# askerlee/segtran

Measured on NVIDIA H100. Metric: voxels/sec fwd+bwd Segtran3d BraTS 112^3 bs=4 hot path, higher is better.
Workload: dtype tf32

## Files before the change

### include/segtran_b200.h

```cpp
#ifndef SEGTRAN_B200_H_
#define SEGTRAN_B200_H_

#include <stddef.h>
#include <stdint.h>

#ifdef __cplusplus
extern "C" {
#endif

#define SX_VERSION 1

enum { SX_F32 = 0, SX_BF16 = 1 };
enum { SX_OP_TF32 = 0, SX_OP_BF16 = 1 };
enum { SX_MAJOR_K = 0, SX_MAJOR_MN = 1 };
enum { SX_BIAS_NONE = 0, SX_BIAS_N = 1, SX_BIAS_M = 2 };
enum { SX_ACT_NONE = 0, SX_ACT_GELU = 1,
       SX_ACT_GELU_BWD = 2  };

int sx_version(void);
const char* sx_last_error(void);
int sx_device_info(int* sm_count, int* cc_major, int* cc_minor);

typedef struct {
  const void* ptr;
// ... 12 lines not shown
  int32_t c_dtype;
  int32_t round_tf32;
  int64_t ldc, c_stride_z0, c_stride_z1;
  float alpha;
  int32_t bias_mode;
  const float* bias;
  int64_t bias_stride_z0, bias_stride_z1;
  int32_t act;
  int32_t accumulate;
  void* preact;
  int32_t split_k;
  int32_t _pad2;
  float* amax;
  float drop_p;
  uint32_t _pad3;
  uint64_t drop_seed;
  const uint64_t* drop_seed_dev;
  const float* addend;
  float* part;
  int64_t part_floats;
} sx_gemm_args;

int sx_gemm(const sx_gemm_args* args, void* stream);

typedef struct {
  const float* table;
  int32_t pd, R;
  int32_t grid[3];
  float w;
} sx_posbias;

typedef struct {
  int32_t B, M, U1, U2, d;
  int32_t round_tf32;
  const float* Q;
  int64_t q_ld, q_bstride;
  const float* K;
  int64_t k_ld, k_bstride;
  float alpha, clip;
  float* P;
  float* S;
  int64_t ldp;
  float* lse;
  float* rowmax;
  float* stat;
  float* diag;
// ... 203 lines not shown
```

### segtran_b200/_lib.py

```python
from __future__ import annotations

import ctypes as C
import os

_HERE = os.path.dirname(os.path.abspath(__file__))
LIB_PATH = os.path.join(_HERE, "libsegtran_b200.so")

SX_F32, SX_BF16 = 0, 1
SX_OP_TF32, SX_OP_BF16 = 0, 1
SX_MAJOR_K, SX_MAJOR_MN = 0, 1
SX_BIAS_NONE, SX_BIAS_N, SX_BIAS_M = 0, 1, 2
SX_ACT_NONE, SX_ACT_GELU, SX_ACT_GELU_BWD = 0, 1, 2
SX_SCHED_WARMUP_LINEAR, SX_SCHED_WARMUP_CONSTANT = 0, 1
SX_CONSIST_BCE, SX_CONSIST_MARGIN = 0, 1
SX_HEAD_DMAP_NONE, SX_HEAD_DMAP_INTERP, SX_HEAD_DMAP_UNFOLD = 0, 1, 2


class SxError(RuntimeError):
    pass


class sx_operand(C.Structure):
    _fields_ = [("ptr", C.c_void_p), ("major", C.c_int32), ("_pad", C.c_int32), ("ld", C.c_int64),
                ("stride_z0", C.c_int64), ("stride_z1", C.c_int64)]


class sx_gemm_args(C.Structure):
    _fields_ = [("op_dtype", C.c_int32), ("M", C.c_int32), ("N", C.c_int32), ("K", C.c_int32), ("Z0", C.c_int32),
                ("Z1", C.c_int32), ("A", sx_operand), ("B", sx_operand), ("C", C.c_void_p), ("c_dtype", C.c_int32),
                ("round_tf32", C.c_int32), ("ldc", C.c_int64), ("c_stride_z0", C.c_int64), ("c_stride_z1", C.c_int64),
                ("alpha", C.c_float), ("bias_mode", C.c_int32), ("bias", C.c_void_p), ("bias_stride_z0", C.c_int64),
                ("bias_stride_z1", C.c_int64), ("act", C.c_int32), ("accumulate", C.c_int32), ("preact", C.c_void_p),
                ("split_k", C.c_int32), ("_pad2", C.c_int32), ("amax", C.c_void_p), ("drop_p", C.c_float),
                ("_pad3", C.c_uint32), ("drop_seed", C.c_uint64), ("drop_seed_dev", C.c_void_p), ("addend", C.c_void_p),
                ("part", C.c_void_p), ("part_floats", C.c_int64)]


class sx_posbias(C.Structure):
    _fields_ = [("table", C.c_void_p), ("pd", C.c_int32), ("R", C.c_int32), ("grid", C.c_int32 * 3), ("w", C.c_float)]


class sx_attn_probs_args(C.Structure):
    _fields_ = [("B", C.c_int32), ("M", C.c_int32), ("U1", C.c_int32), ("U2", C.c_int32), ("d", C.c_int32),
                ("round_tf32", C.c_int32), ("Q", C.c_void_p), ("q_ld", C.c_int64), ("q_bstride", C.c_int64),
                ("K", C.c_void_p), ("k_ld", C.c_int64), ("k_bstride", C.c_int64), ("alpha", C.c_float),
                ("clip", C.c_float), ("P", C.c_void_p), ("S", C.c_void_p), ("ldp", C.c_int64), ("lse", C.c_void_p),
                ("rowmax", C.c_void_p), ("stat", C.c_void_p), ("diag", C.c_void_p), ("drop_p", C.c_float),
                ("_pad", C.c_uint32), ("drop_seed", C.c_uint64), ("drop_seed_dev", C.c_void_p), ("posbias", sx_posbias)]


class sx_consist_args(C.Structure):
    _fields_ = [("B", C.c_int32), ("N", C.c_int32), ("A", C.c_int32), ("K", C.c_int32), ("variant", C.c_int32),
                ("round_r", C.c_int32), ("Xo", C.c_void_p), ("xo_ld", C.c_int64), ("xo_bstride", C.c_int64),
                ("Xt", C.c_void_p), ("xt_ld", C.c_int64), ("xt_bstride", C.c_int64), ("X", C.c_void_p),
                ("x_ld", C.c_int64), ("x_bstride", C.c_int64), ("F", C.c_void_p), ("mu", C.c_void_p), ("R", C.c_void_p),
                ("ldr", C.c_int64), ("out", C.c_void_p), ("cap", C.c_void_p), ("cap_scale", C.c_float),
                ("_pad", C.c_int32), ("part", C.c_void_p), ("part_floats", C.c_int64)]


class sx_head_dropout_args(C.Structure):
    _fields_ = [("src", C.c_void_p), ("B", C.c_int32), ("Fs", C.c_int32), ("Ds", C.c_int32), ("Fo", C.c_int32),
                ("HW", C.c_int64), ("Dk", C.c_int32), ("dmap", C.c_int32), ("K", C.c_int32), ("_pad", C.c_int32),
                ("Wc", C.c_void_p), ("bc", C.c_void_p), ("p", C.c_float), ("_pad2", C.c_uint32), ("seed", C.c_uint64),
                ("seed_dev", C.c_void_p), ("part", C.c_void_p), ("part_floats", C.c_int64)]


class sx_resample_grid(C.Structure):
    _fields_ = [("lin", C.c_int32 * 3), ("lout", C.c_int32 * 3), ("ratio", C.c_float * 3)]


_P, _I, _L, _F, _U64, _D = C.c_void_p, C.c_int32, C.c_int64, C.c_float, C.c_uint64, C.c_double

_PROTOS = {
    "sx_gemm": [C.POINTER(sx_gemm_args), _P],
    "sx_gemm_debug_set": [C.c_char_p, _L],
    "sx_attn_probs_fwd": [C.POINTER(sx_attn_probs_args), _P],
    "sx_attn_consist_fwd": [C.POINTER(sx_consist_args), _P],
    "sx_attn_consist_bwd": [C.POINTER(sx_consist_args), _P, _P, _I, _I, _L, _L, _P, _P, _P, _L, _L, _P],
    "sx_clamp_if": [_P, _L, _I, _L, _P, _F, _P, _L, _P, _L, _P],
    "sx_reduce_max": [_P, _L, _P, _P],
    "sx_pos_lsinu_fwd": [_P, _P, _L, _I, _P, _P, _I, _P, _P],
    "sx_pos_lsinu_bwd": [_P, _P, _L, _I, _P, _P, _I, _P, _P, _P, _P, _P, _L, _P],
    "sx_prologue_fwd": [_P, _L, _I, _I, _P, _P, _P, _I, _L, _F, _P, _F, _U64, _P, _P, _I, _P, _P],
    "sx_prologue_bwd": [_P, _P, _L, _I, _I, _P, _P, _P, _I, _L, _F, _P, _F, _U64, _P, _P, _P, _P, _P, _P, _P, _P, _L, _P],
    "sx_softmax_fwd": [_P, _L, _I, _L, _P, _F, _F, _U64, _P, _P, _L, _I, _P, _P, _P],
    "sx_softmax_bwd": [_P, _L, _P, _L, _P, _L, _I, _P, _F, _F, _U64, _P, _L, _P, _L, _I, _P],
    "sx_softmax_posbias_fwd": [_P, _L, _I, _L, _P, _F, _F, _U64, _P, _P, _L, _I, _P, _P, C.POINTER(sx_posbias), _P],
    "sx_softmax_posbias_bwd": [_P, _L, _P, _L, _P, _L, _I, _P, _F, _F, _U64, _P, _L, _P, _L, _I, C.POINTER(sx_posbias),
                               _P, _P, _L, _P],
    "sx_layernorm_fwd": [_P, _L, _I, _P, _P, _P, _I, _P, _P],
    "sx_layernorm_bwd": [_P, _P, _L, _I, _P, _P, _P, _I, _P, _P, _P, _L, _P],
    "sx_ln_softaggr_fwd": [_P, _I, _I, _I, _I, _P, _P, _P, _P, _F, _U64, _P, _P, _P, _P, _P],
    "sx_ln_softaggr_bwd": [_P, _P, _I, _I, _I, _I, _P, _P, _P, _F, _U64, _P, _P, _P, _P, _I, _P, _P, _P, _P, _P, _L, _P],
    "sx_softaggr_fwd": [_P, _I, _I, _I, _I, _P, _P, _P, _P, _P],
    "sx_softaggr_bwd": [_P, _P, _I, _I, _I, _I, _P, _P, _P, _P, _P],
    "sx_gelu_bwd": [_P, _P, _L, _F, _U64, _P, _P, _I, _P],
    "sx_seed_derive": [_P, _U64, _P, _P],
# ... 48 lines not shown
    global _lib
    if _lib is None:
        if not os.path.isfile(LIB_PATH):
            raise SxError("segtran_b200: %s is missing - run `python -c 'import __graft_entry__ as g; g.build()'` "
                          "or `make` at the repo root (there is no CPU / PyTorch fallback)" % LIB_PATH)
        l = C.CDLL(LIB_PATH)
        l.sx_version.restype = C.c_int
        l.sx_last_error.restype = C.c_char_p
        l.sx_device_info.argtypes = [C.POINTER(C.c_int)] * 3
        l.sx_device_info.restype = C.c_int
        for name, at in _PROTOS.items():
            f = getattr(l, name)
            f.argtypes = at
            f.restype = C.c_int
        _lib = l
    return _lib


def check(rc, what):
    if rc != 0:
        raise SxError("%s failed (rc=%d): %s" % (what, rc, lib().sx_last_error().decode("utf-8", "replace")))


_LAUNCHES = {"sx_pos_lsinu_bwd": 3, "sx_ln_softaggr_bwd": 2, "sx_prologue_bwd": 3, "sx_layernorm_bwd": 3, "sx_gemm_debug_set": 0,
             "sx_attn_probs_fwd": 2, "sx_colsum_batched": 2, "sx_dot": 2, "sx_head_contract_bwd_weight": 2,
             "sx_softmax_posbias_bwd": 2, "sx_attn_consist_fwd": 2, "sx_head_dropout_bwd": 2, "sx_edt_sq": 3}
launch_count = 0
_hook = None


def set_hook(h):
    global _hook
    _hook = h


def call(name, *args):
    global launch_count
    launch_count += _LAUNCHES.get(name, 1)
    if _hook is None:
        check(getattr(lib(), name)(*args), name)
    else:
        with _hook(name, args):
            check(getattr(lib(), name)(*args), name)
```

### segtran_b200/csrc/sx_gemm.cu

```cuda
#include <algorithm>
#include <string>

#include "sx_common.cuh"
#include "sx_tc.cuh"

namespace {
using namespace sxtc;

constexpr int NUM_THREADS = 384;
constexpr int STAGES = 4;
constexpr int XPOSE_WARPS = 3;
constexpr int BN_WIDE = 256;

template <int ES, bool A_MN, bool B_MN, int BN_T>
struct Plan {
  static_assert(BN_T == BN || (BN_T == BN_WIDE && ES == 4 && !A_MN && !B_MN),
                "sx_gemm: the 256-column tile is instantiated for K-major tf32 operands only");
  static constexpr int B_BYTES = BN_T * BKB;
  static constexpr int STAGE_BYTES = A_STAGE_BYTES + B_BYTES;
  static constexpr bool XA = ES == 4 && A_MN, XB = ES == 4 && B_MN;
  static constexpr bool XPOSE = XA || XB;
  static constexpr int RAW_BYTES = (XA ? A_STAGE_BYTES : 0) + (XB ? B_STAGE_BYTES : 0);
  static constexpr int RAW_SLOTS = !XPOSE ? 0 : (XA && XB ? 3 : 4);
  static constexpr int DIRECT_BYTES = STAGE_BYTES - RAW_BYTES;
  static constexpr int SMEM = STAGES * STAGE_BYTES + RAW_SLOTS * RAW_BYTES + 1024  + 256 ;
  static_assert(SMEM <= 227 * 1024, "sx_gemm: shared memory plan exceeds 227 KB");
  static_assert(!XPOSE || (A_STAGE_BYTES == 16384 && B_STAGE_BYTES == 16384 && BM == 128 && BN == 128),
                "sx_gemm: the transposer assumes 128-row, 16 KB tf32 operand tiles");
};

struct GemmParams {
  int M, N, K, Z0, Z1;
  int tiles_m, tiles_n, split_k, kb_per_split, num_kb, total_tiles;
  int z1_loop;
  float* part;
  int a_uses_z0, a_uses_z1, b_uses_z0, b_uses_z1;
  void* C;
  int c_bf16;
  int round_tf32;
  int c_vec_ok;
  long long ldc, c_sz0, c_sz1;
  float alpha;
  int bias_mode;
  const float* bias;
  long long bias_sz0, bias_sz1;
  int act;
  int accumulate;
  void* preact;
  float* amax;
  float drop_p;
  unsigned long long drop_seed;
  const unsigned long long* drop_seed_dev;
  const float* addend;
  int stream_out;
};

__device__ __forceinline__ void xpose_load(uint32_t src, int b, float4 (&v)[4]) {
  const int c = b & 7, kc = c ^ ((b >> 3) & 7);
  const uint32_t s = src + (b >> 6) * 4096;
#pragma unroll
  for (int e = 0; e < 4; ++e) {
    const int k = 4 * kc + e;
    asm volatile("ld.shared.v4.f32 {%0, %1, %2, %3}, [%4];"
                 : "=f"(v[e].x), "=f"(v[e].y), "=f"(v[e].z), "=f"(v[e].w)
                 : "r"(s + k * 128 + ((c ^ (k & 7)) << 4)) : "memory");
  }
}
__device__ __forceinline__ void xpose_store(uint32_t dst, int b, const float4 (&v)[4]) {
  const int c = b & 7, kc = c ^ ((b >> 3) & 7);
  const int r0 = (b >> 6) * 32 + 4 * c;
  auto st = [&](int i, float x, float y, float z, float w) {
    asm volatile("st.shared.v4.f32 [%0], {%1, %2, %3, %4};"
                 ::"r"(dst + (r0 + i) * 128 + ((kc ^ ((r0 + i) & 7)) << 4)), "f"(x), "f"(y), "f"(z), "f"(w) : "memory");
  };
  st(0, v[0].x, v[1].x, v[2].x, v[3].x);
  st(1, v[0].y, v[1].y, v[2].y, v[3].y);
  st(2, v[0].z, v[1].z, v[2].z, v[3].z);
  st(3, v[0].w, v[1].w, v[2].w, v[3].w);
}

template <int ES, bool A_MN, bool B_MN, int BN_T>
__global__ void __launch_bounds__(NUM_THREADS, 1)
sx_gemm_kernel(const __grid_constant__ CUtensorMap tmA, const __grid_constant__ CUtensorMap tmB, const GemmParams p) {
  using PL = Plan<ES, A_MN, B_MN, BN_T>;
  constexpr bool kTF32 = (ES == 4);
  constexpr bool WIDE = BN_T == BN_WIDE;
  constexpr int STAGE_BYTES = PL::STAGE_BYTES;
  constexpr bool XA = PL::XA, XB = PL::XB;
  constexpr int BK = BKB / ES;
  constexpr int MN_BOX = BKB / ES;
  constexpr int MN_BOX_BYTES = BK * BKB;
  constexpr int KSTEPS = 4;

  extern __shared__ uint8_t smem_raw[];
  uint8_t* smem = reinterpret_cast<uint8_t*>((reinterpret_cast<uintptr_t>(smem_raw) + 1023) & ~uintptr_t(1023));
  uint8_t* raw = smem + STAGES * STAGE_BYTES;
  uint64_t* bars = reinterpret_cast<uint64_t*>(raw + PL::RAW_SLOTS * PL::RAW_BYTES);
  uint64_t* full_bar = bars;
  uint64_t* empty_bar = bars + STAGES;
  uint64_t* raw_full = bars + 2 * STAGES;
  uint64_t* raw_empty = raw_full + PL::RAW_SLOTS;

  const int warp = threadIdx.x >> 5;
  const int lane = threadIdx.x & 31;
  const int wg = threadIdx.x >> 7;

  if (threadIdx.x == 0) {
    sx::tma_prefetch_desc(&tmA);
    sx::tma_prefetch_desc(&tmB);
    for (int s = 0; s < STAGES; ++s) {
      sx::mbar_init(&full_bar[s], (PL::DIRECT_BYTES ? 1 : 0) + (PL::XPOSE ? XPOSE_WARPS : 0));
      sx::mbar_init(&empty_bar[s], 2);
    }
    for (int s = 0; s < PL::RAW_SLOTS; ++s) {
      sx::mbar_init(&raw_full[s], 1);
      sx::mbar_init(&raw_empty[s], XPOSE_WARPS);
    }
    sx::fence_barrier_init();
  }
  __syncthreads();

  auto decode = [&](int t, int& z0, int& z1, int& mb, int& nb, int& ks) {
    nb = t % p.tiles_n; t /= p.tiles_n;
    mb = t % p.tiles_m; t /= p.tiles_m;
// ... 302 lines not shown
      if (p.amax) {
#pragma unroll
        for (int h = 0; h < 2; ++h)
          if (row0 + 8 * h + tr < p.M) {
#pragma unroll
            for (int j = 0; j < 4; ++j)
#pragma unroll
              for (int e = 0; e < 2; ++e)
                if (col0 + 8 * j + tc + e < p.N) tmax = fmaxf(tmax, f[4 * j + 2 * h + e]);
          }
      }
      if (!WIDE && p.split_k > 1) {
        float* pt = p.part + ((((long long)z1 * p.Z0 + z0) * p.tiles_m + mb) * p.tiles_n + nb) * p.split_k * (BM * BN) +
                    (long long)ks * (BM * BN);
#pragma unroll
        for (int h = 0; h < 2; ++h)
#pragma unroll
          for (int j = 0; j < 4; ++j)
            *reinterpret_cast<float2*>(pt + (row0 - mb * BM + 8 * h + tr) * BN + (col0 - nb * BN) + 8 * j + tc) =
                make_float2(f[4 * j + 2 * h], f[4 * j + 2 * h + 1]);
      } else {
        store_frag(p.C, f, zoff, row0, col0, p.accumulate != 0);
      }
      if constexpr (WIDE) {
#pragma unroll
        for (int i = 0; i < BN_T / 2 - 16; ++i) acc[i] = acc[i + 16];
      }
    }
    if (p.amax) {
      tmax = sx::warp_max(tmax);
      if (lane == 0 && tmax > -3.0e38f) sx::atomic_max_float(p.amax, tmax);
    }
  }
}

__global__ void split_reduce_kernel(const GemmParams p) {
  const long long total = (long long)p.total_tiles / p.split_k * (BM * BN);
  for (long long i = (long long)blockIdx.x * blockDim.x + threadIdx.x; i < total; i += (long long)gridDim.x * blockDim.x) {
    const int e = (int)(i % (BM * BN));
    long long t = i / (BM * BN);
    const int nb = (int)(t % p.tiles_n); t /= p.tiles_n;
    const int mb = (int)(t % p.tiles_m); t /= p.tiles_m;
    const int z0 = (int)(t % p.Z0), z1 = (int)(t / p.Z0);
    const int row = mb * BM + e / BN, col = nb * BN + e % BN;
    if (row >= p.M || col >= p.N) continue;
    const float* pt = p.part + (i / (BM * BN)) * p.split_k * (BM * BN) + e;
// ... 14 lines not shown
  kern<<<grid, NUM_THREADS, bytes, st>>>(ta, tb, p);
  SX_CHECK_CUDA(cudaGetLastError());
  if (p.split_k > 1) {
    const long long n = (long long)p.total_tiles / p.split_k * (BM * BN);
    split_reduce_kernel<<<(int)std::min<long long>(sx_ceil_div(n, 256), 65535), 256, 0, st>>>(p);
    SX_CHECK_CUDA(cudaGetLastError());
  }
  return 0;
}

}

extern "C" int sx_gemm_debug_set(const char* key, int64_t value) {
  std::string k(key);
  if (k == "max_ctas") g_max_ctas = value;
  else if (k == "wide_tiles") g_wide_tiles = value < 0 ? -1 : (value ? 1 : 0);
  else {
    sx_set_error("sx_gemm_debug_set: unknown key %s", key);
    return -1;
  }
  return 0;
}

extern "C" int sx_gemm(const sx_gemm_args* a, void* stream) {
  SX_REQUIRE(a != nullptr, "sx_gemm: null args");
  SX_REQUIRE(a->M > 0 && a->N > 0 && a->K > 0 && a->Z0 > 0 && a->Z1 > 0, "sx_gemm: bad shape M=%d N=%d K=%d Z=%dx%d",
             a->M, a->N, a->K, a->Z0, a->Z1);
  SX_REQUIRE(a->op_dtype == SX_OP_TF32 || a->op_dtype == SX_OP_BF16, "sx_gemm: bad op_dtype %d", a->op_dtype);
  SX_REQUIRE(a->C != nullptr && a->A.ptr != nullptr && a->B.ptr != nullptr, "sx_gemm: null pointer");
  const int es = a->op_dtype == SX_OP_TF32 ? 4 : 2;
  const int bk = BKB / es;
  const int sms = sm_count_cached();
  SX_REQUIRE(sms > 0, "sx_gemm: no CUDA device (this library has no CPU fallback)");

  GemmParams p{};
  p.M = a->M; p.N = a->N; p.K = a->K; p.Z0 = a->Z0; p.Z1 = a->Z1;
  p.tiles_m = sx_ceil_div(a->M, BM);
  p.tiles_n = sx_ceil_div(a->N, BN);
  p.num_kb = sx_ceil_div(a->K, bk);
  const bool fold_z1 = a->Z1 > 1 && a->c_stride_z1 == 0;
  SX_REQUIRE(!fold_z1 || (a->accumulate && !a->bias && !a->addend && a->act == SX_ACT_NONE && !a->preact && a->drop_p == 0.f),
             "sx_gemm: a z1-reduced output needs accumulate=1 and a linear epilogue without bias");
  p.z1_loop = fold_z1 ? a->Z1 : 1;
  p.Z1 = fold_z1 ? 1 : a->Z1;
  int split = a->split_k < 1 ? 1 : a->split_k;
  if (split > p.num_kb) split = p.num_kb;
  {
// ... 14 lines not shown
  const bool wide_legal = es == 4 && !amn && !bmn && p.split_k == 1;
  const long long wide_tt = (long long)p.tiles_m * sx_ceil_div(a->N, BN_WIDE) * a->Z0 * p.Z1;
  const bool wide = wide_legal && (g_wide_tiles == 1 || (g_wide_tiles < 0 && a->N > BN && 2 * wide_tt > sms));
  if (wide) p.tiles_n = sx_ceil_div(a->N, BN_WIDE);
  const long long tt = (long long)p.tiles_m * p.tiles_n * p.split_k * a->Z0 * p.Z1;
  SX_REQUIRE(tt < (1ll << 30), "sx_gemm: too many tiles");
  p.total_tiles = (int)tt;
  p.a_uses_z0 = a->A.stride_z0 != 0; p.a_uses_z1 = a->A.stride_z1 != 0;
  p.b_uses_z0 = a->B.stride_z0 != 0; p.b_uses_z1 = a->B.stride_z1 != 0;
  p.C = a->C; p.c_bf16 = a->c_dtype == SX_BF16; p.round_tf32 = a->round_tf32;
  p.ldc = a->ldc; p.c_sz0 = a->c_stride_z0; p.c_sz1 = a->c_stride_z1;
  p.c_vec_ok = ((reinterpret_cast<uintptr_t>(a->C) & 7) == 0) && (a->ldc % 2 == 0) && (a->c_stride_z0 % 2 == 0) &&
               (a->c_stride_z1 % 2 == 0) && (!a->preact || (reinterpret_cast<uintptr_t>(a->preact) & 7) == 0) &&
               (!a->addend || (reinterpret_cast<uintptr_t>(a->addend) & 7) == 0);
  p.alpha = a->alpha; p.bias_mode = a->bias ? a->bias_mode : SX_BIAS_NONE; p.bias = a->bias;
  p.bias_sz0 = a->bias_stride_z0; p.bias_sz1 = a->bias_stride_z1;
  p.act = a->act; p.accumulate = a->accumulate; p.preact = a->preact; p.amax = a->amax;
  p.addend = a->addend;
  SX_REQUIRE(a->act != SX_ACT_GELU_BWD || (a->preact && a->c_dtype == SX_F32 && p.split_k == 1 && !a->accumulate),
             "sx_gemm: SX_ACT_GELU_BWD needs the fp32 pre-activation in `preact`, fp32 C, split_k=1, accumulate=0");
  SX_REQUIRE(!a->addend || (p.split_k == 1 && !a->accumulate && a->c_dtype == SX_F32), "sx_gemm: addend needs split_k=1, accumulate=0, fp32 C");
  p.drop_p = a->drop_p; p.drop_seed = a->drop_seed;
  p.drop_seed_dev = reinterpret_cast<const unsigned long long*>(a->drop_seed_dev);
  {
    const double out_bytes = (double)a->M * a->N * a->Z0 * a->Z1 * (p.c_bf16 ? 2 : 4) * (a->preact ? 2 : 1);
    p.stream_out = out_bytes > 25.0 * 1024 * 1024;
  }

  CUtensorMap ta, tb;
  int rc = make_map(&ta, a->A, es, a->M, a->K, a->Z0, a->Z1, BM, "A");
  if (rc) return rc;
  rc = make_map(&tb, a->B, es, a->N, a->K, a->Z0, a->Z1, wide ? BN_WIDE : BN, "B");
  if (rc) return rc;

  int grid = p.total_tiles < sms ? p.total_tiles : sms;
  if (g_max_ctas > 0 && grid > g_max_ctas) grid = (int)g_max_ctas;
  p.part = a->part;
  cudaStream_t st = reinterpret_cast<cudaStream_t>(stream);
  if (wide) return launch<4, false, false, BN_WIDE>(ta, tb, p, grid, st);
  if (es == 4) {
    if (!amn && !bmn) return launch<4, false, false>(ta, tb, p, grid, st);
    if (!amn && bmn) return launch<4, false, true>(ta, tb, p, grid, st);
    if (amn && !bmn) return launch<4, true, false>(ta, tb, p, grid, st);
    return launch<4, true, true>(ta, tb, p, grid, st);
  }
  if (!amn && !bmn) return launch<2, false, false>(ta, tb, p, grid, st);
  if (!amn && bmn) return launch<2, false, true>(ta, tb, p, grid, st);
  if (amn && !bmn) return launch<2, true, false>(ta, tb, p, grid, st);
  return launch<2, true, true>(ta, tb, p, grid, st);
}
```

### segtran_b200/ops.py

```python
from __future__ import annotations

import ctypes as C
import math
import os
from typing import Optional

import numpy as np
import torch

from . import _lib as L

_PRECISION = "tf32"


def set_precision(p: str):
    global _PRECISION
    if p not in ("tf32", "tf32x3", "bf16"):
        raise ValueError("unsupported precision %r (this build implements 'tf32', 'tf32x3' and 'bf16')" % (p,))
    _PRECISION = p
    _bf16_cache.clear()


def get_precision() -> str:
    return _PRECISION
# ... 245 lines not shown
        t = _part_bufs[key] = torch.empty(_PART_FLOATS, device=device, dtype=torch.float32)
    return t.data_ptr(), t.numel()


def _pick_split_k(M, N, K, Z, bk=32, sms=132, epi=10):
    tiles = ((M + 127) // 128) * ((N + 127) // 128) * Z
    nkb = (K + bk - 1) // bk
    if tiles >= 2 * sms or nkb < 16:
        return 1
    best, best_cost = 1, None
    for sk in range(1, max(1, nkb // 8) + 1):
        rounds = (tiles * sk + sms - 1) // sms
        cost = rounds * ((nkb + sk - 1) // sk + epi * (1 if sk == 1 else 2))
        if best_cost is None or cost < best_cost:
            best, best_cost = sk, cost
    return best


def _gemm_nt_1(a: torch.Tensor, b: torch.Tensor, *, out: Optional[torch.Tensor] = None, alpha: float = 1.0,
               bias: Optional[torch.Tensor] = None, bias_mode: int = L.SX_BIAS_N, gelu: bool = False,
               preact: Optional[torch.Tensor] = None, accumulate: bool = False, split_k: Optional[int] = None,
               amax: Optional[torch.Tensor] = None, drop_p: float = 0.0, seed: int = 0, round_out: bool = True,
               reduce_z1: bool = False, addend: Optional[torch.Tensor] = None,
               gelu_bwd: Optional[torch.Tensor] = None) -> torch.Tensor:
    _req_cuda(a, b, out, bias, preact, amax)
    if a.dtype != torch.float32 or b.dtype != torch.float32:
        raise L.SxError("gemm_nt: fp32 operands expected (precision policy %s)" % _PRECISION)
    a4, b4 = _as4(a), _as4(b)
    M, K = a4.shape[-2:]
    N, K2 = b4.shape[-2:]
    if K != K2:
        raise L.SxError("gemm_nt: K mismatch %d vs %d" % (K, K2))
    Z1 = max(a4.shape[0], b4.shape[0])
    Z0 = max(a4.shape[1], b4.shape[1])
    for t in (a4, b4):
        if t.shape[0] not in (1, Z1) or t.shape[1] not in (1, Z0):
            raise L.SxError("gemm_nt: batch dims do not broadcast")
    oz1 = 1 if reduce_z1 else Z1
    fresh = out is None
    linear_epi = (not gelu) and preact is None and drop_p == 0.0 and amax is None and gelu_bwd is None
    if split_k is None:
        split_k = _pick_split_k(M, N, K, Z0 * Z1) if (linear_epi and (fresh or accumulate or reduce_z1)) else 1
    if fresh:
        if accumulate or reduce_z1 or split_k > 1:
            out = _zeros((oz1, Z0, M, N), a.device)
        else:
            out = torch.empty((oz1, Z0, M, N), device=a.device, dtype=torch.float32)
    o4 = _as4(out)
    if o4.shape[-2:] != (M, N) or o4.stride(-1) != 1:
        raise L.SxError("gemm_nt: bad output view %s %s" % (tuple(o4.shape), o4.stride()))
    g = L.sx_gemm_args()
    g.op_dtype = L.SX_OP_TF32
    if _PRECISION == "bf16":
        a4, b4 = _bf16_view(a4), _bf16_view(b4)
        g.op_dtype = L.SX_OP_BF16
    g.M, g.N, g.K, g.Z0, g.Z1 = M, N, K, Z0, Z1
    g.A = _operand(a4, Z1, Z0, "A")
    g.B = _operand(b4, Z1, Z0, "B")
    g.C = o4.data_ptr()
    g.c_dtype = L.SX_F32
    round_after = round_out and _PRECISION == "tf32" and (split_k > 1 or accumulate or reduce_z1)
    g.round_tf32 = 1 if (round_out and _PRECISION == "tf32" and not round_after) else 0
    g.ldc = o4.stride(-2)
# ... 8 lines not shown
        g.bias_mode = bias_mode
        g.bias_stride_z0 = b4b.stride(1) if b4b.shape[1] > 1 else 0
        g.bias_stride_z1 = b4b.stride(0) if b4b.shape[0] > 1 else 0
    g.act = L.SX_ACT_GELU if gelu else L.SX_ACT_NONE
    if gelu_bwd is not None:
        if gelu or preact is not None or tuple(gelu_bwd.shape[-2:]) != (M, N) or gelu_bwd.stride() != out.stride():
            raise L.SxError("gemm_nt: gelu_bwd needs the pre-activation in the output's layout and no other activation")
        g.act = L.SX_ACT_GELU_BWD
        g.preact = gelu_bwd.data_ptr()
    g.split_k = split_k
    if split_k > 1:
        g.part, g.part_floats = _part_args(a.device)
    g.accumulate = 1 if (accumulate or reduce_z1 or split_k > 1) else 0
    if preact is not None:
        g.preact = preact.data_ptr()
    if amax is not None:
        g.amax = amax.data_ptr()
    g.drop_p = drop_p
    g.drop_seed, g.drop_seed_dev = _seed_args(seed)
    if addend is not None:
        if addend.dtype != torch.float32 or tuple(addend.shape[-2:]) != (M, N) or _as4(addend).stride() != o4.stride():
            raise L.SxError("gemm_nt: addend must be an fp32 tensor in the output's layout")
        g.addend = addend.data_ptr()
    L.call("sx_gemm", C.byref(g), _stream())
    if round_after and fresh:
        L.call("sx_convert", out.data_ptr(), L.SX_F32, out.numel(), out.data_ptr(), L.SX_F32, 1, _stream())
    return out


def gemm_nt(a: torch.Tensor, b: torch.Tensor, *, out: Optional[torch.Tensor] = None, alpha: float = 1.0,
            bias: Optional[torch.Tensor] = None, bias_mode: int = L.SX_BIAS_N, gelu: bool = False,
            preact: Optional[torch.Tensor] = None, accumulate: bool = False, split_k: Optional[int] = None,
            amax: Optional[torch.Tensor] = None, drop_p: float = 0.0, seed: int = 0, round_out: bool = True,
            reduce_z1: bool = False, gelu_bwd: Optional[torch.Tensor] = None,
            addend: Optional[torch.Tensor] = None, tag: str = "big") -> torch.Tensor:
    if not _three_pass(tag):
        return _gemm_nt_1(a, b, out=out, alpha=alpha, bias=bias, bias_mode=bias_mode, gelu=gelu, preact=preact,
                          accumulate=accumulate, split_k=split_k, amax=amax, drop_p=drop_p, seed=seed,
                          round_out=round_out, reduce_z1=reduce_z1, gelu_bwd=gelu_bwd, addend=addend)
    _req_cuda(a, b)
    return _gemm_nt_1(_split_cat(a, 0), _split_cat(b, 1), out=out, alpha=alpha, bias=bias, bias_mode=bias_mode, gelu=gelu,
                      preact=preact, accumulate=accumulate, split_k=split_k, amax=amax, drop_p=drop_p, seed=seed,
                      round_out=round_out, reduce_z1=reduce_z1, gelu_bwd=gelu_bwd, addend=addend)


def _split_cat(t: torch.Tensor, role: int) -> torch.Tensor:
    t4 = _as4(t)
    Z1, Z0, R, K = t4.shape
    Kp = _pad4(K)
    out = torch.empty((Z1, Z0, R, 3 * Kp), device=t.device, dtype=torch.float32)
    L.call("sx_split_tf32_cat", t4.data_ptr(), Z1, Z0, R, K, t4.stride(0), t4.stride(1), t4.stride(2), t4.stride(3), Kp, role,
           out.data_ptr(), _stream())
    return out


def _pad4(n: int) -> int:
    return (n + 3) // 4 * 4


def _rowpad_empty(shape, device) -> torch.Tensor:
    Lr = shape[-1]
    buf = torch.empty(tuple(shape[:-1]) + (_pad4(Lr),), device=device, dtype=torch.float32)
# ... 31 lines not shown
        return x
    y = torch.empty_like(x)
    L.call("sx_convert", x.data_ptr(), L.SX_F32, x.numel(), y.data_ptr(), L.SX_F32, 1, _stream())
    return y


_KMAJOR_COPIES = os.environ.get("SEGTRAN_KMAJOR_COPIES", "1") != "0"


def set_kmajor_copies(on: bool):
    global _KMAJOR_COPIES
    _KMAJOR_COPIES = bool(on)


def _kmajor_copies(tag: str = "big") -> bool:
    return _KMAJOR_COPIES and _PRECISION == "tf32" and not _three_pass(tag)


def _transposed(x: torch.Tensor, Z: int, R: int, Cd: int) -> torch.Tensor:
    x = x.contiguous()
    y = _rowpad_empty((Z, Cd, R), x.device)
    L.call("sx_transpose", x.data_ptr(), Z, R, Cd, y.stride(1), y.data_ptr(), _stream())
    return y


def _weight_t(Wr: torch.Tensor, Z: int, O: int, I: int) -> torch.Tensor:
    if _kmajor_copies():
        return _transposed(Wr, Z, O, I)
    return Wr.reshape(Z, O, I).transpose(-1, -2)


def colsum(x2d: torch.Tensor, out: Optional[torch.Tensor] = None) -> torch.Tensor:
    if out is None:
        out = _zeros((x2d.shape[1],), x2d.device)
    L.call("sx_colsum_batched", x2d.data_ptr(), 1, 0, 1, 0, x2d.shape[0], x2d.shape[1], x2d.stride(0), out.data_ptr(),
           *_part_args(x2d.device), _stream())
    return out


class _Linear(torch.autograd.Function):

    @staticmethod
    def forward(ctx, x, W, b, gelu, drop_p, seed, tag, round_y, addend):
        shp = x.shape
        x2 = x.reshape(-1, shp[-1])
        if not x2.is_contiguous():
# ... 294 lines not shown
        ctx.leaf = table
        return P

    @staticmethod
    def backward(ctx, dP):
        S, lse, amax, _table = ctx.saved_tensors
        clip, drop_p, seed, ldp, pb_geom = ctx.meta
        dS, dT = softmax_backward(dP, S, lse, amax, clip, drop_p, seed, ldp, ctx.leaf, pb_geom, ctx.needs_input_grad[6])
        return dS, None, None, None, None, None, dT, None


class _AttnPV(torch.autograd.Function):

    @staticmethod
    def forward(ctx, P, v, M, tag, round_out, heads):
        B, _, U1, U2 = P.shape
        Fd = v.shape[-1] // M
        P = _rowpad(P)
        if heads:
            U = torch.empty((B, U1, M * Fd), device=P.device, dtype=torch.float32)
            gemm_nt(P, _head_cols(v, B, U2, M, Fd, _kmajor_copies(tag)), out=U.view(B, U1, M, Fd).permute(0, 2, 1, 3),
                    tag=tag, round_out=round_out)
        else:
            vv = v.view(B, U2, M, Fd).permute(0, 2, 3, 1)
            U = torch.empty((B, M, U1, Fd), device=P.device, dtype=torch.float32)
            gemm_nt(P, vv, out=U, tag=tag, round_out=round_out)
        ctx.save_for_backward(P, v)
        ctx.meta = (M, Fd, heads)
        ctx.tag = tag
        return U

    @staticmethod
    def backward(ctx, dU):
        P, v = ctx.saved_tensors
        M, Fd, heads = ctx.meta
        B, _, U1, U2 = P.shape
        dU = dU.contiguous()
        dP = dv = None
        if heads:
            if ctx.needs_input_grad[0]:
                dP = _rowpad_empty((B, M, U1, U2), P.device)
                gemm_nt(_head_rows(dU, B, U1, M, Fd), _head_rows(v, B, U2, M, Fd), out=dP, round_out=False, tag=ctx.tag)
            if ctx.needs_input_grad[1]:
                dv = torch.empty_like(v)
                gemm_nt(P.transpose(-1, -2), _head_cols(dU, B, U1, M, Fd, False),
                        out=dv.view(B, U2, M, Fd).permute(0, 2, 1, 3), round_out=False, tag=ctx.tag)
            return dP, dv, None, None, None, None
        dP, dv = _pv_grads(dU, P, v, M, Fd, ctx.needs_input_grad[0], ctx.needs_input_grad[1], ctx.tag)
        return dP, dv, None, None, None, None


def _pv_grads(dU, P, v, M, Fd, need_p, need_v, tag):
    B, _, U1, U2 = P.shape
    dP = dv = None
    if need_p:
        dP = _rowpad_empty((B, M, U1, U2), P.device)
        gemm_nt(dU, v.view(B, U2, M, Fd).permute(0, 2, 1, 3), out=dP, round_out=False, tag=tag)
    if need_v:
        dv = torch.empty_like(v)
        gemm_nt(P.transpose(-1, -2), dU.transpose(-1, -2), out=dv.view(B, U2, M, Fd).permute(0, 2, 1, 3),
                round_out=False, tag=tag)
    return dP, dv


class _FoldedValueBank(torch.autograd.Function):

    @staticmethod
    def forward(ctx, a, Wv, Wm, M, tag):
        B, A, Cd = a.shape
        Fd = Wm.shape[0]
        a2 = a.reshape(B * A, Cd)
        if not a2.is_contiguous():
            a2 = a2.contiguous()
        x3 = _three_pass(tag)
        Wvr = (Wv.contiguous() if x3 else round_tf32(Wv)).view(M, 1, Fd, Cd)
        Wmr = Wm.contiguous() if x3 else round_tf32(Wm)
        Wf = gemm_nt(Wmr.view(1, 1, Fd, Fd), Wvr.transpose(-1, -2), tag=tag, round_out=not x3)
        Vp = gemm_nt(a2, Wf.view(M * Fd, Cd), tag=tag)[0, 0]
        if x3 and _PRECISION == "tf32":
            Wf, Wvr, Wmr = round_tf32(Wf), round_tf32(Wv).view(M, 1, Fd, Cd), round_tf32(Wm)
        ctx.save_for_backward(a2, Wf, Wvr, Wmr)
        ctx.meta = (B, A, Cd, Fd, M)
        ctx.leaves = (Wv, Wm)
        return Vp.view(B, A, M * Fd)
# ... 10 lines not shown
        if ctx.needs_input_grad[0]:
            da = gemm_nt(d2, _weight_t(Wf, 1, M * Fd, Cd)[0], round_out=False)[0, 0].view(B, A, Cd)
        if ctx.needs_input_grad[1] or ctx.needs_input_grad[2]:
            dWf = gemm_nt(d2.t(), a2.t(), round_out=False).view(M, 1, Fd, Cd)
            if ctx.needs_input_grad[2]:
                dWm = _param_grad(Wm, dWf, Wvr, (1, 1, Fd, Fd), reduce_z1=True)
            if ctx.needs_input_grad[1]:
                dWv = _param_grad(Wv, Wmr.t().view(1, 1, Fd, Fd), dWf.transpose(-1, -2), (M, 1, Fd, Cd))
        return da, dWv, dWm, None, None


def folded_value_bank(a, Wv, Wm, M, tag="small"):
    return _FoldedValueBank.apply(a, Wv, Wm, M, tag)


def _group_linear_fwd(G, Wo, bo):
    M, Fd = G.shape[1], G.shape[3]
    Wr = round_tf32(Wo).reshape(M, Fd, Fd)
    Y = torch.empty_like(G)
    gemm_nt(G, Wr.unsqueeze(0), out=Y, bias=bo.reshape(1, M, Fd), round_out=False)
    return Y, Wr


def _group_linear_param_grads(dY, G, Wo, bo, need_w, need_b):
    B, M, N, Fd = G.shape
    dW = db = None
    if need_w:
        dW = _param_grad(Wo, dY.transpose(-1, -2), G.transpose(-1, -2), (1, M, Fd, Fd), reduce_z1=True)
    if need_b:
        tgt = _grad_target(bo)
        buf = tgt if tgt is not None else _zeros((M * Fd,), G.device)
        L.call("sx_colsum_batched", dY.data_ptr(), B, M * N * Fd, M, N * Fd, N, Fd, Fd, buf.data_ptr(),
               *_part_args(dY.device), _stream())
        db = None if tgt is not None else buf
    return dW, db


class _AttnPVGeluGroupLinear(torch.autograd.Function):

    @staticmethod
    def forward(ctx, P, v, M, bm, drop_p, seed, Wo, bo):
        B, _, U1, U2 = P.shape
        Fd = v.shape[-1] // M
        P = _rowpad(P)
        G = torch.empty((B, M, U1, Fd), device=P.device, dtype=torch.float32)
        H = torch.empty_like(G)
        gemm_nt(P, _head_cols(v, B, U2, M, Fd, _kmajor_copies()), out=G, bias=bm, gelu=True, preact=H, drop_p=drop_p,
                seed=seed)
        Y, Wr = _group_linear_fwd(G, Wo, bo)
        ctx.save_for_backward(P, v, H, G, Wr)
        ctx.meta = (M, Fd, drop_p, seed)
        ctx.leaves = (bm, Wo, bo)
        return Y

    @staticmethod
    def backward(ctx, dY):
        P, v, H, G, Wr = ctx.saved_tensors
        M, Fd, drop_p, seed = ctx.meta
        bm, Wo, bo = ctx.leaves
        dY = dY.contiguous()
        dbm_buf = dbm = None
        if bm is not None and ctx.needs_input_grad[3]:
            tgt = _grad_target(bm)
            dbm_buf = tgt if tgt is not None else _zeros((Fd,), dY.device)
            dbm = None if tgt is not None else dbm_buf
        dH = torch.empty_like(H)
        gemm_nt(dY, _weight_t(Wr, M, Fd, Fd).unsqueeze(0), out=dH, gelu_bwd=H, drop_p=drop_p, seed=seed)
        if dbm_buf is not None:
            colsum(dH.view(-1, Fd), out=dbm_buf)
        dW, dbo = _group_linear_param_grads(dY, G, Wo, bo, ctx.needs_input_grad[6], ctx.needs_input_grad[7])
        dP, dv = _pv_grads(dH, P, v, M, Fd, ctx.needs_input_grad[0], ctx.needs_input_grad[1], "big")
        return dP, dv, None, dbm, None, None, dW, dbo


def attn_pv_gelu_group_linear(P, v, M, bm, drop_p, seed, Wo, bo):
    return _AttnPVGeluGroupLinear.apply(P, v, M, bm, drop_p, seed, Wo, bo)


_ATTN_FUSION = True


def set_attn_fusion(on: bool):
    global _ATTN_FUSION
    _ATTN_FUSION = bool(on)


def attn_fusion_enabled() -> bool:
    return _ATTN_FUSION and _PRECISION == "tf32"


def _pb_args(posbias):
    if posbias is None:
        return None, None
    return _posbias_table(posbias), (posbias.R, posbias.grid, posbias.w)
# ... 1110 lines not shown
```

Measured before the change: 508.2 million.

## Emit transposed GEMM outputs from the epilogue for K-major backward operands

Adds an optional second, transposed output to the tf32 K-major GEMM epilogue, staged through extra shared memory with named barriers, so the GELU group-linear forward and backward can write G and dH in token-major layout directly. Backward weight and value gradients then consume K-major operands instead of MN-major views that need the in-kernel transposer, and large PV products use K-major copies via a size heuristic. The cost is an extra output write, more shared memory per CTA, and explicit transpose copies of P and dY in some paths.

```diff
diff --git a/include/segtran_b200.h b/include/segtran_b200.h
--- a/include/segtran_b200.h
+++ b/include/segtran_b200.h
@@ -58,6 +58,13 @@
 } sx_gemm_args;
 
 int sx_gemm(const sx_gemm_args* args, void* stream);
+
+typedef struct {
+  float* ct;
+  int64_t ldct, ct_stride_z0, ct_stride_z1;
+} sx_gemm_tout;
+
+int sx_gemm_set_tout(const sx_gemm_tout* tout);
 
 typedef struct {
   const float* table;
diff --git a/segtran_b200/_lib.py b/segtran_b200/_lib.py
--- a/segtran_b200/_lib.py
+++ b/segtran_b200/_lib.py
@@ -34,6 +34,10 @@
                 ("split_k", C.c_int32), ("_pad2", C.c_int32), ("amax", C.c_void_p), ("drop_p", C.c_float),
                 ("_pad3", C.c_uint32), ("drop_seed", C.c_uint64), ("drop_seed_dev", C.c_void_p), ("addend", C.c_void_p),
                 ("part", C.c_void_p), ("part_floats", C.c_int64)]
+
+
+class sx_gemm_tout(C.Structure):
+    _fields_ = [("ct", C.c_void_p), ("ldct", C.c_int64), ("ct_stride_z0", C.c_int64), ("ct_stride_z1", C.c_int64)]
 
 
 class sx_posbias(C.Structure):
@@ -73,6 +77,7 @@
 
 _PROTOS = {
     "sx_gemm": [C.POINTER(sx_gemm_args), _P],
+    "sx_gemm_set_tout": [C.POINTER(sx_gemm_tout)],
     "sx_gemm_debug_set": [C.c_char_p, _L],
     "sx_attn_probs_fwd": [C.POINTER(sx_attn_probs_args), _P],
     "sx_attn_consist_fwd": [C.POINTER(sx_consist_args), _P],
@@ -167,7 +172,7 @@
         raise SxError("%s failed (rc=%d): %s" % (what, rc, lib().sx_last_error().decode("utf-8", "replace")))
 
 
-_LAUNCHES = {"sx_pos_lsinu_bwd": 3, "sx_ln_softaggr_bwd": 2, "sx_prologue_bwd": 3, "sx_layernorm_bwd": 3, "sx_gemm_debug_set": 0,
+_LAUNCHES = {"sx_pos_lsinu_bwd": 3, "sx_ln_softaggr_bwd": 2, "sx_prologue_bwd": 3, "sx_layernorm_bwd": 3, "sx_gemm_debug_set": 0, "sx_gemm_set_tout": 0,
              "sx_attn_probs_fwd": 2, "sx_colsum_batched": 2, "sx_dot": 2, "sx_head_contract_bwd_weight": 2,
              "sx_softmax_posbias_bwd": 2, "sx_attn_consist_fwd": 2, "sx_head_dropout_bwd": 2, "sx_edt_sq": 3}
 launch_count = 0
diff --git a/segtran_b200/csrc/sx_gemm.cu b/segtran_b200/csrc/sx_gemm.cu
--- a/segtran_b200/csrc/sx_gemm.cu
+++ b/segtran_b200/csrc/sx_gemm.cu
@@ -11,6 +11,8 @@
 constexpr int STAGES = 4;
 constexpr int XPOSE_WARPS = 3;
 constexpr int BN_WIDE = 256;
+constexpr int CT_LD = 68;
+constexpr int CT_WG_FLOATS = 32 * CT_LD;
 
 template <int ES, bool A_MN, bool B_MN, int BN_T>
 struct Plan {
@@ -23,7 +25,9 @@
   static constexpr int RAW_BYTES = (XA ? A_STAGE_BYTES : 0) + (XB ? B_STAGE_BYTES : 0);
   static constexpr int RAW_SLOTS = !XPOSE ? 0 : (XA && XB ? 3 : 4);
   static constexpr int DIRECT_BYTES = STAGE_BYTES - RAW_BYTES;
-  static constexpr int SMEM = STAGES * STAGE_BYTES + RAW_SLOTS * RAW_BYTES + 1024  + 256 ;
+  static constexpr bool CT = ES == 4 && !A_MN && !B_MN;
+  static constexpr int CT_BYTES = CT ? 2 * CT_WG_FLOATS * 4 : 0;
+  static constexpr int SMEM = STAGES * STAGE_BYTES + RAW_SLOTS * RAW_BYTES + 1024  + 256  + CT_BYTES;
   static_assert(SMEM <= 227 * 1024, "sx_gemm: shared memory plan exceeds 227 KB");
   static_assert(!XPOSE || (A_STAGE_BYTES == 16384 && B_STAGE_BYTES == 16384 && BM == 128 && BN == 128),
                 "sx_gemm: the transposer assumes 128-row, 16 KB tf32 operand tiles");
@@ -53,6 +57,8 @@
   const unsigned long long* drop_seed_dev;
   const float* addend;
   int stream_out;
+  float* ct;
+  long long ldct, ct_sz0, ct_sz1;
 };
 
 __device__ __forceinline__ void xpose_load(uint32_t src, int b, float4 (&v)[4]) {
@@ -78,6 +84,8 @@
   st(2, v[0].z, v[1].z, v[2].z, v[3].z);
   st(3, v[0].w, v[1].w, v[2].w, v[3].w);
 }
+
+__device__ __forceinline__ void named_bar_sync(int id) { asm volatile("bar.sync %0, 128;" ::"r"(id) : "memory"); }
 
 template <int ES, bool A_MN, bool B_MN, int BN_T>
 __global__ void __launch_bounds__(NUM_THREADS, 1)
@@ -100,6 +108,7 @@
   uint64_t* empty_bar = bars + STAGES;
   uint64_t* raw_full = bars + 2 * STAGES;
   uint64_t* raw_empty = raw_full + PL::RAW_SLOTS;
+  float* ct_stage = reinterpret_cast<float*>(reinterpret_cast<uint8_t*>(bars) + 256);
 
   const int warp = threadIdx.x >> 5;
   const int lane = threadIdx.x & 31;
@@ -448,6 +457,38 @@
       } else {
         store_frag(p.C, f, zoff, row0, col0, p.accumulate != 0);
       }
+      if constexpr (PL::CT) {
+        if (p.ct) {
+          float* cs = ct_stage + cw * CT_WG_FLOATS;
+          named_bar_sync(1 + cw);
+#pragma unroll
+          for (int j = 0; j < 4; ++j)
+#pragma unroll
+            for (int h = 0; h < 2; ++h)
+#pragma unroll
+              for (int e = 0; e < 2; ++e) cs[(8 * j + tc + e) * CT_LD + wq * 16 + 8 * h + tr] = f[4 * j + 2 * h + e];
+          named_bar_sync(1 + cw);
+          const int m0 = mb * BM + cw * 64;
+          const long long ctz = (long long)z1 * p.ct_sz1 + (long long)z0 * p.ct_sz0;
+#pragma unroll
+          for (int i = 0; i < 4; ++i) {
+            const int v = wtid + 128 * i, n = v >> 4, r = (v & 15) * 4;
+            const int gn = col0 + n, gm = m0 + r;
+            if (gn < p.N && gm < p.M) {
+              const float4 x = *reinterpret_cast<const float4*>(cs + n * CT_LD + r);
+              float* o = p.ct + ctz + (long long)gn * p.ldct + gm;
+              if (gm + 3 < p.M) {
+                if (p.stream_out) __stcs(reinterpret_cast<float4*>(o), x);
+                else *reinterpret_cast<float4*>(o) = x;
+              } else {
+                o[0] = x.x;
+                if (gm + 1 < p.M) o[1] = x.y;
+                if (gm + 2 < p.M) o[2] = x.z;
+              }
+            }
+          }
+        }
+      }
       if constexpr (WIDE) {
 #pragma unroll
         for (int i = 0; i < BN_T / 2 - 16; ++i) acc[i] = acc[i + 16];
@@ -508,7 +549,7 @@
   return 0;
 }
 
-extern "C" int sx_gemm(const sx_gemm_args* a, void* stream) {
+static int gemm_run(const sx_gemm_args* a, const sx_gemm_tout* t, void* stream) {
   SX_REQUIRE(a != nullptr, "sx_gemm: null args");
   SX_REQUIRE(a->M > 0 && a->N > 0 && a->K > 0 && a->Z0 > 0 && a->Z1 > 0, "sx_gemm: bad shape M=%d N=%d K=%d Z=%dx%d",
              a->M, a->N, a->K, a->Z0, a->Z1);
@@ -569,8 +610,19 @@
   SX_REQUIRE(!a->addend || (p.split_k == 1 && !a->accumulate && a->c_dtype == SX_F32), "sx_gemm: addend needs split_k=1, accumulate=0, fp32 C");
   p.drop_p = a->drop_p; p.drop_seed = a->drop_seed;
   p.drop_seed_dev = reinterpret_cast<const unsigned long long*>(a->drop_seed_dev);
+  if (t) {
+    SX_REQUIRE(t->ct != nullptr, "sx_gemm: null ct");
+    SX_REQUIRE(es == 4 && !amn && !bmn, "sx_gemm: ct needs tf32 operands, both K-major");
+    SX_REQUIRE(p.split_k == 1 && !a->accumulate && a->c_dtype == SX_F32,
+               "sx_gemm: ct needs split_k=1, accumulate=0, fp32 C");
+    SX_REQUIRE((reinterpret_cast<uintptr_t>(t->ct) & 15) == 0 && t->ldct % 4 == 0 && t->ct_stride_z0 % 4 == 0 &&
+                   t->ct_stride_z1 % 4 == 0 && t->ldct >= a->M,
+               "sx_gemm: ct must be 16-byte aligned with ldct >= M and ldct, z strides multiples of 4");
+    p.ct = t->ct; p.ldct = t->ldct; p.ct_sz0 = t->ct_stride_z0; p.ct_sz1 = t->ct_stride_z1;
+  }
   {
-    const double out_bytes = (double)a->M * a->N * a->Z0 * a->Z1 * (p.c_bf16 ? 2 : 4) * (a->preact ? 2 : 1);
+    const double out_bytes =
+        (double)a->M * a->N * a->Z0 * a->Z1 * (p.c_bf16 ? 2 : 4) * (1 + (a->preact ? 1 : 0) + (t ? 1 : 0));
     p.stream_out = out_bytes > 25.0 * 1024 * 1024;
   }
 
@@ -596,3 +648,17 @@
   if (amn && !bmn) return launch<2, true, false>(ta, tb, p, grid, st);
   return launch<2, true, true>(ta, tb, p, grid, st);
 }
+
+static thread_local sx_gemm_tout g_tout{};
+
+extern "C" int sx_gemm_set_tout(const sx_gemm_tout* t) {
+  g_tout = t ? *t : sx_gemm_tout{};
+  SX_REQUIRE(t == nullptr || t->ct != nullptr, "sx_gemm_set_tout: null ct");
+  return 0;
+}
+
+extern "C" int sx_gemm(const sx_gemm_args* a, void* stream) {
+  const sx_gemm_tout t = g_tout;
+  g_tout = sx_gemm_tout{};
+  return gemm_run(a, t.ct ? &t : nullptr, stream);
+}
diff --git a/segtran_b200/ops.py b/segtran_b200/ops.py
--- a/segtran_b200/ops.py
+++ b/segtran_b200/ops.py
@@ -291,7 +291,7 @@
                preact: Optional[torch.Tensor] = None, accumulate: bool = False, split_k: Optional[int] = None,
                amax: Optional[torch.Tensor] = None, drop_p: float = 0.0, seed: int = 0, round_out: bool = True,
                reduce_z1: bool = False, addend: Optional[torch.Tensor] = None,
-               gelu_bwd: Optional[torch.Tensor] = None) -> torch.Tensor:
+               gelu_bwd: Optional[torch.Tensor] = None, ct: Optional[torch.Tensor] = None) -> torch.Tensor:
     _req_cuda(a, b, out, bias, preact, amax)
     if a.dtype != torch.float32 or b.dtype != torch.float32:
         raise L.SxError("gemm_nt: fp32 operands expected (precision policy %s)" % _PRECISION)
@@ -307,7 +307,7 @@
             raise L.SxError("gemm_nt: batch dims do not broadcast")
     oz1 = 1 if reduce_z1 else Z1
     fresh = out is None
-    linear_epi = (not gelu) and preact is None and drop_p == 0.0 and amax is None and gelu_bwd is None
+    linear_epi = (not gelu) and preact is None and drop_p == 0.0 and amax is None and gelu_bwd is None and ct is None
     if split_k is None:
         split_k = _pick_split_k(M, N, K, Z0 * Z1) if (linear_epi and (fresh or accumulate or reduce_z1)) else 1
     if fresh:
@@ -362,6 +362,16 @@
         if addend.dtype != torch.float32 or tuple(addend.shape[-2:]) != (M, N) or _as4(addend).stride() != o4.stride():
             raise L.SxError("gemm_nt: addend must be an fp32 tensor in the output's layout")
         g.addend = addend.data_ptr()
+    if ct is not None:
+        t4 = _as4(ct)
+        if ct.dtype != torch.float32 or tuple(t4.shape[-2:]) != (N, M) or t4.stride(-1) != 1 or round_after:
+            raise L.SxError("gemm_nt: ct must be an fp32 [..., N, M] view with m contiguous, on a single-pass product")
+        t = L.sx_gemm_tout()
+        t.ct = t4.data_ptr()
+        t.ldct = t4.stride(-2)
+        t.ct_stride_z0 = t4.stride(1) if t4.shape[1] > 1 else 0
+        t.ct_stride_z1 = t4.stride(0) if t4.shape[0] > 1 else 0
+        L.call("sx_gemm_set_tout", C.byref(t))
     L.call("sx_gemm", C.byref(g), _stream())
     if round_after and fresh:
         L.call("sx_convert", out.data_ptr(), L.SX_F32, out.numel(), out.data_ptr(), L.SX_F32, 1, _stream())
@@ -373,11 +383,13 @@
             preact: Optional[torch.Tensor] = None, accumulate: bool = False, split_k: Optional[int] = None,
             amax: Optional[torch.Tensor] = None, drop_p: float = 0.0, seed: int = 0, round_out: bool = True,
             reduce_z1: bool = False, gelu_bwd: Optional[torch.Tensor] = None,
-            addend: Optional[torch.Tensor] = None, tag: str = "big") -> torch.Tensor:
+            addend: Optional[torch.Tensor] = None, tag: str = "big", ct: Optional[torch.Tensor] = None) -> torch.Tensor:
     if not _three_pass(tag):
         return _gemm_nt_1(a, b, out=out, alpha=alpha, bias=bias, bias_mode=bias_mode, gelu=gelu, preact=preact,
                           accumulate=accumulate, split_k=split_k, amax=amax, drop_p=drop_p, seed=seed,
-                          round_out=round_out, reduce_z1=reduce_z1, gelu_bwd=gelu_bwd, addend=addend)
+                          round_out=round_out, reduce_z1=reduce_z1, gelu_bwd=gelu_bwd, addend=addend, ct=ct)
+    if ct is not None:
+        raise L.SxError("gemm_nt: ct needs a single-pass product")
     _req_cuda(a, b)
     return _gemm_nt_1(_split_cat(a, 0), _split_cat(b, 1), out=out, alpha=alpha, bias=bias, bias_mode=bias_mode, gelu=gelu,
                       preact=preact, accumulate=accumulate, split_k=split_k, amax=amax, drop_p=drop_p, seed=seed,
@@ -455,6 +467,11 @@
     y = _rowpad_empty((Z, Cd, R), x.device)
     L.call("sx_transpose", x.data_ptr(), Z, R, Cd, y.stride(1), y.data_ptr(), _stream())
     return y
+
+
+def _token_kmajor(M: int, N: int, K: int, Z: int, tag: str = "big") -> bool:
+    return _kmajor_copies(tag) and min(M, N) >= 512 and K >= 1024 and \
+        2 * ((M + 127) // 128) * ((N + 255) // 256) * Z > 132
 
 
 def _weight_t(Wr: torch.Tensor, Z: int, O: int, I: int) -> torch.Tensor:
@@ -795,7 +812,7 @@
             gemm_nt(P, _head_cols(v, B, U2, M, Fd, _kmajor_copies(tag)), out=U.view(B, U1, M, Fd).permute(0, 2, 1, 3),
                     tag=tag, round_out=round_out)
         else:
-            vv = v.view(B, U2, M, Fd).permute(0, 2, 3, 1)
+            vv = _head_cols(v, B, U2, M, Fd, _token_kmajor(U1, Fd, U2, B * M, tag))
             U = torch.empty((B, M, U1, Fd), device=P.device, dtype=torch.float32)
             gemm_nt(P, vv, out=U, tag=tag, round_out=round_out)
         ctx.save_for_backward(P, v)
@@ -823,7 +840,7 @@
         return dP, dv, None, None, None, None
 
 
-def _pv_grads(dU, P, v, M, Fd, need_p, need_v, tag):
+def _pv_grads(dU, P, v, M, Fd, need_p, need_v, tag, dUt=None):
     B, _, U1, U2 = P.shape
     dP = dv = None
     if need_p:
@@ -831,8 +848,15 @@
         gemm_nt(dU, v.view(B, U2, M, Fd).permute(0, 2, 1, 3), out=dP, round_out=False, tag=tag)
     if need_v:
         dv = torch.empty_like(v)
-        gemm_nt(P.transpose(-1, -2), dU.transpose(-1, -2), out=dv.view(B, U2, M, Fd).permute(0, 2, 1, 3),
-                round_out=False, tag=tag)
+        if dUt is None and _token_kmajor(U2, Fd, U1, B * M, tag):
+            dUt = _transposed(dU, B * M, U1, Fd).unflatten(0, (B, M))
+        if dUt is not None:
+            Pt = _transposed(P, B * M, U1, U2).unflatten(0, (B, M))
+            gemm_nt(Pt, dUt, out=dv.view(B, U2, M, Fd).permute(0, 2, 1, 3), round_out=False, tag=tag)
+            del Pt
+        else:
+            gemm_nt(P.transpose(-1, -2), dU.transpose(-1, -2), out=dv.view(B, U2, M, Fd).permute(0, 2, 1, 3),
+                    round_out=False, tag=tag)
     return dP, dv
 
 
@@ -889,14 +913,19 @@
     return Y, Wr
 
 
-def _group_linear_param_grads(dY, G, Wo, bo, need_w, need_b):
-    B, M, N, Fd = G.shape
+def _group_linear_param_grads(dY, G, Wo, bo, need_w, need_b, Gt=None):
+    B, M, N, Fd = dY.shape
     dW = db = None
     if need_w:
-        dW = _param_grad(Wo, dY.transpose(-1, -2), G.transpose(-1, -2), (1, M, Fd, Fd), reduce_z1=True)
+        if Gt is not None:
+            dYt = _transposed(dY, B * M, N, Fd).unflatten(0, (B, M))
+            dW = _param_grad(Wo, dYt, Gt, (1, M, Fd, Fd), reduce_z1=True)
+            del dYt
+        else:
+            dW = _param_grad(Wo, dY.transpose(-1, -2), G.transpose(-1, -2), (1, M, Fd, Fd), reduce_z1=True)
     if need_b:
         tgt = _grad_target(bo)
-        buf = tgt if tgt is not None else _zeros((M * Fd,), G.device)
+        buf = tgt if tgt is not None else _zeros((M * Fd,), dY.device)
         L.call("sx_colsum_batched", dY.data_ptr(), B, M * N * Fd, M, N * Fd, N, Fd, Fd, buf.data_ptr(),
                *_part_args(dY.device), _stream())
         db = None if tgt is not None else buf
@@ -912,18 +941,20 @@
         P = _rowpad(P)
         G = torch.empty((B, M, U1, Fd), device=P.device, dtype=torch.float32)
         H = torch.empty_like(G)
+        kt = _token_kmajor(Fd, Fd, U1, M) and _token_kmajor(U2, Fd, U1, B * M)
+        Gt = _rowpad_empty((B, M, Fd, U1), P.device) if kt else None
         gemm_nt(P, _head_cols(v, B, U2, M, Fd, _kmajor_copies()), out=G, bias=bm, gelu=True, preact=H, drop_p=drop_p,
-                seed=seed)
+                seed=seed, ct=Gt)
         Y, Wr = _group_linear_fwd(G, Wo, bo)
-        ctx.save_for_backward(P, v, H, G, Wr)
-        ctx.meta = (M, Fd, drop_p, seed)
+        ctx.save_for_backward(P, v, H, Gt if kt else G, Wr)
+        ctx.meta = (M, Fd, drop_p, seed, kt)
         ctx.leaves = (bm, Wo, bo)
         return Y
 
     @staticmethod
     def backward(ctx, dY):
         P, v, H, G, Wr = ctx.saved_tensors
-        M, Fd, drop_p, seed = ctx.meta
+        M, Fd, drop_p, seed, kt = ctx.meta
         bm, Wo, bo = ctx.leaves
         dY = dY.contiguous()
         dbm_buf = dbm = None
@@ -932,11 +963,14 @@
             dbm_buf = tgt if tgt is not None else _zeros((Fd,), dY.device)
             dbm = None if tgt is not None else dbm_buf
         dH = torch.empty_like(H)
-        gemm_nt(dY, _weight_t(Wr, M, Fd, Fd).unsqueeze(0), out=dH, gelu_bwd=H, drop_p=drop_p, seed=seed)
+        B, _, U1, _ = P.shape
+        dHt = _rowpad_empty((B, M, Fd, U1), dY.device) if kt and ctx.needs_input_grad[1] else None
+        gemm_nt(dY, _weight_t(Wr, M, Fd, Fd).unsqueeze(0), out=dH, gelu_bwd=H, drop_p=drop_p, seed=seed, ct=dHt)
         if dbm_buf is not None:
             colsum(dH.view(-1, Fd), out=dbm_buf)
-        dW, dbo = _group_linear_param_grads(dY, G, Wo, bo, ctx.needs_input_grad[6], ctx.needs_input_grad[7])
-        dP, dv = _pv_grads(dH, P, v, M, Fd, ctx.needs_input_grad[0], ctx.needs_input_grad[1], "big")
+        dW, dbo = _group_linear_param_grads(dY, None if kt else G, Wo, bo, ctx.needs_input_grad[6],
+                                            ctx.needs_input_grad[7], Gt=G if kt else None)
+        dP, dv = _pv_grads(dH, P, v, M, Fd, ctx.needs_input_grad[0], ctx.needs_input_grad[1], "big", dUt=dHt)
         return dP, dv, None, dbm, None, None, dW, dbo
 
 
```

After: 531.1 million (median of 6 runs). 1.05x the previous value.
